# constantinpape/torch-em

Measured on AMD Instinct MI355X. Metric: voxels/sec fwd+bwd, UNet3d 1x128^3 bs=2, higher is better.
Workload: dtype f32-class (forward convs on normalised activations: fp32 operands split into 2 fp16 terms = 22 mantissa bits, lo plane scaled by 2^12 with its own fp32 accumulator, 3 fp16 MFMAs per product; other forward convs 3 bf16 terms / 6 MFMAs; data-gradient convs 2 bf16 terms / 3 MFMAs (16-bit products); WEI

## Files before the change

### torch_em_amd/csrc/capi.hip

```cpp
#include "tem_common.h"
#include "conv_internal.h"
#include "tem_act.h"
#include <stdarg.h>
#include <string.h>

static thread_local char g_err[512] = "";

void tem_set_error(const char* fmt, ...) {
    va_list ap;
    va_start(ap, fmt);
    vsnprintf(g_err, sizeof(g_err), fmt, ap);
    va_end(ap);
}

extern "C" const char* tem_last_error(void) { return g_err; }

struct TemOption {
    const char* name;
    long long def;
};
static const TemOption g_opt_table[TEM_OPT_COUNT] = {
    {"wgrad_zs", 3},
    {"wgrad_zs_persist", 1},
    {"wgrad_sums", 1},
    {"wgrad_sums_min_mb", 128},
    {"fwd_persistent", -1},
    {"conv_fwd_variant", -1},
    {"conv1x1_stream", 1},
    {"fwd_ksplit_chunks", 0},
    {"wgrad_cus", 256},
    {"upsample_generic", 0},
    {"team_min_units", 0},
    {"zr_splitk", 1},
    {"zr_wide", 1},
    {"zr_tile_blocks", 1},
    {"dice_vox", 1},
    {"upsample2_ch8", 1},
    {"pool_vec8", 2},
    {"fp32_zr", 1},
};
static long long g_opt_val[TEM_OPT_COUNT];
static bool g_opt_set[TEM_OPT_COUNT];

long long tem_option(int id) {
    if (id < 0 || id >= TEM_OPT_COUNT) return 0;
    return __atomic_load_n(&g_opt_set[id], __ATOMIC_RELAXED) ? __atomic_load_n(&g_opt_val[id], __ATOMIC_RELAXED)
                                                            : g_opt_table[id].def;
}
static int opt_find(const char* name) {
    if (!name) return -1;
    for (int i = 0; i < TEM_OPT_COUNT; ++i)
        if (!strcmp(name, g_opt_table[i].name)) return i;
    return -1;
}
extern "C" int tem_set_option(const char* name, int64_t value) {
    const int id = opt_find(name);
    TEM_REQUIRE(id >= 0, "tem_set_option: unknown option '%s'", name ? name : "(null)");
    __atomic_store_n(&g_opt_val[id], (long long)value, __ATOMIC_RELAXED);
    __atomic_store_n(&g_opt_set[id], true, __ATOMIC_RELAXED);
    return TEM_OK;
}
extern "C" int tem_get_option(const char* name, int64_t* value) {
    const int id = opt_find(name);
    TEM_REQUIRE(id >= 0 && value, "tem_get_option: unknown option '%s'", name ? name : "(null)");
    *value = (int64_t)tem_option(id);
    return TEM_OK;
}
extern "C" int tem_version(void) { return 100; }

extern "C" int tem_device_cus(void) {
    int dev = 0;
    if (hipGetDevice(&dev) != hipSuccess) return TEM_ELAUNCH;
    hipDeviceProp_t prop;
    if (hipGetDeviceProperties(&prop, dev) != hipSuccess) return TEM_ELAUNCH;
    return prop.multiProcessorCount;
}

#define TT_V 64
#define TT_C 32

__global__ __launch_bounds__(256) void k_nchw_to_nhwc(const float* __restrict__ src, float* __restrict__ dst,
                                                      int64_t dst_ld, int C, int64_t V, int64_t vtiles, int ctiles) {
    __shared__ float tile[TT_C][TT_V + 1];
    int64_t ntiles = vtiles * ctiles;
    int n = blockIdx.y;
    for (int64_t t = blockIdx.x; t < ntiles; t += gridDim.x) {
        int ct = (int)(t % ctiles);
        int64_t vt = t / ctiles;
        int64_t v0 = vt * TT_V;
        int c0 = ct * TT_C;
        for (int i = threadIdx.x; i < TT_C * TT_V; i += 256) {
            int c = i / TT_V, v = i % TT_V;
            float val = 0.f;
            if (c0 + c < C && v0 + v < V) val = src[((int64_t)n * C + c0 + c) * V + v0 + v];
            tile[c][v] = val;
        }
        __syncthreads();
        for (int i = threadIdx.x; i < TT_C * TT_V; i += 256) {
            int v = i / TT_C, c = i % TT_C;
            if (c0 + c < C && v0 + v < V) dst[((int64_t)n * V + v0 + v) * dst_ld + c0 + c] = tile[c][v];
        }
        __syncthreads();
    }
}

__global__ __launch_bounds__(256) void k_nhwc_to_nchw(const float* __restrict__ src, int64_t src_ld,
                                                      float* __restrict__ dst, int C, int64_t V, int64_t vtiles,
                                                      int ctiles) {
    __shared__ float tile[TT_C][TT_V + 1];
    int64_t ntiles = vtiles * ctiles;
    int n = blockIdx.y;
    for (int64_t t = blockIdx.x; t < ntiles; t += gridDim.x) {
        int ct = (int)(t % ctiles);
        int64_t vt = t / ctiles;
        int64_t v0 = vt * TT_V;
        int c0 = ct * TT_C;
        for (int i = threadIdx.x; i < TT_C * TT_V; i += 256) {
            int v = i / TT_C, c = i % TT_C;
            float val = 0.f;
            if (c0 + c < C && v0 + v < V) val = src[((int64_t)n * V + v0 + v) * src_ld + c0 + c];
            tile[c][v] = val;
        }
        __syncthreads();
        for (int i = threadIdx.x; i < TT_C * TT_V; i += 256) {
            int c = i / TT_V, v = i % TT_V;
            if (c0 + c < C && v0 + v < V) dst[((int64_t)n * C + c0 + c) * V + v0 + v] = tile[c][v];
        }
        __syncthreads();
    }
}

extern "C" int tem_nchw_to_nhwc(const float* src, float* dst, int64_t dst_ld, int N, int C, int64_t V,
                                tem_stream_t stream) {
    TEM_REQUIRE(src && dst && N > 0 && C > 0 && V > 0 && dst_ld >= C, "tem_nchw_to_nhwc: bad arguments");
    int64_t vtiles = tem_cdiv(V, TT_V);
    int ctiles = (int)tem_cdiv(C, TT_C);
    int64_t nt = vtiles * ctiles;
    dim3 grid((unsigned)(nt > 4096 ? 4096 : nt), N);
    hipLaunchKernelGGL(k_nchw_to_nhwc, grid, dim3(256), 0, (hipStream_t)stream, src, dst, dst_ld, C, V, vtiles, ctiles);
    TEM_CHECK_LAUNCH("tem_nchw_to_nhwc");
    return TEM_OK;
}

extern "C" int tem_nhwc_to_nchw(const float* src, int64_t src_ld, float* dst, int N, int C, int64_t V,
                                tem_stream_t stream) {
    TEM_REQUIRE(src && dst && N > 0 && C > 0 && V > 0 && src_ld >= C, "tem_nhwc_to_nchw: bad arguments");
    int64_t vtiles = tem_cdiv(V, TT_V);
    int ctiles = (int)tem_cdiv(C, TT_C);
    int64_t nt = vtiles * ctiles;
    dim3 grid((unsigned)(nt > 4096 ? 4096 : nt), N);
    hipLaunchKernelGGL(k_nhwc_to_nchw, grid, dim3(256), 0, (hipStream_t)stream, src, src_ld, dst, C, V, vtiles, ctiles);
    TEM_CHECK_LAUNCH("tem_nhwc_to_nchw");
    return TEM_OK;
}

#define STD_BLOCKS 256

__global__ __launch_bounds__(256) void k_std_partial(const float* __restrict__ x, int64_t L, double* __restrict__ part) {
    int n = blockIdx.y;
    const float* row = x + (int64_t)n * L;
    double s = 0.0, ss = 0.0;
    for (int64_t i = (int64_t)blockIdx.x * 256 + threadIdx.x; i < L; i += (int64_t)gridDim.x * 256) {
        double v = (double)row[i];
        s += v;
        ss += v * v;
    }
    s = tem_wave_sum_d(s);
    ss = tem_wave_sum_d(ss);
    __shared__ double sh[2][4];
    int w = threadIdx.x >> 6;
    if ((threadIdx.x & 63) == 0) { sh[0][w] = s; sh[1][w] = ss; }
    __syncthreads();
    if (threadIdx.x == 0) {
        part[((int64_t)n * gridDim.x + blockIdx.x) * 2 + 0] = sh[0][0] + sh[0][1] + sh[0][2] + sh[0][3];
        part[((int64_t)n * gridDim.x + blockIdx.x) * 2 + 1] = sh[1][0] + sh[1][1] + sh[1][2] + sh[1][3];
    }
}

__global__ __launch_bounds__(256) void k_std_apply(const float* __restrict__ x, float* __restrict__ y, int64_t L,
                                                   const double* __restrict__ part, int nblk, float eps) {
    int n = blockIdx.y;
    __shared__ float sh_mean, sh_inv;
    if (threadIdx.x == 0) {
        double s = 0.0, ss = 0.0;
        for (int b = 0; b < nblk; ++b) {
            s += part[((int64_t)n * nblk + b) * 2 + 0];
            ss += part[((int64_t)n * nblk + b) * 2 + 1];
        }
        double mean = s / (double)L;
        double var = ss / (double)L - mean * mean;
        if (var < 0.0) var = 0.0;
        sh_mean = (float)mean;
        sh_inv = (float)(1.0 / (sqrt(var) + (double)eps));
    }
    __syncthreads();
    float mean = sh_mean, inv = sh_inv;
    const float* row = x + (int64_t)n * L;
    float* out = y + (int64_t)n * L;
    for (int64_t i = (int64_t)blockIdx.x * 256 + threadIdx.x; i < L; i += (int64_t)gridDim.x * 256)
        out[i] = (row[i] - mean) * inv;
}

extern "C" int tem_standardize(const float* x, float* y, int N, int64_t L, float eps, void* ws, int64_t ws_bytes,
                               tem_stream_t stream) {
    TEM_REQUIRE(x && y && ws && N > 0 && L > 0, "tem_standardize: bad arguments");
    int nblk = (int)(tem_cdiv(L, 256) < STD_BLOCKS ? tem_cdiv(L, 256) : STD_BLOCKS);
    if ((int64_t)N * nblk * 2 * (int64_t)sizeof(double) > ws_bytes) {
        tem_set_error("tem_standardize: workspace too small (%lld bytes needed)",
                      (long long)((int64_t)N * nblk * 2 * sizeof(double)));
        return TEM_EWS;
    }
    hipLaunchKernelGGL(k_std_partial, dim3(nblk, N), dim3(256), 0, (hipStream_t)stream, x, L, (double*)ws);
    hipLaunchKernelGGL(k_std_apply, dim3(nblk, N), dim3(256), 0, (hipStream_t)stream, x, y, L, (const double*)ws, nblk, eps);
    TEM_CHECK_LAUNCH("tem_standardize");
    return TEM_OK;
}

__global__ __launch_bounds__(256) void k_act_bwd(const float* __restrict__ gy, const float* __restrict__ y,
                                                 float* __restrict__ gx, int64_t n, int act) {
    for (int64_t i = (int64_t)blockIdx.x * 256 + threadIdx.x; i < n; i += (int64_t)gridDim.x * 256) {
        float yv = y[i], g = gy[i];
        gx[i] = (act == TEM_ACT_SIGMOID) ? g * yv * (1.f - yv) : ((yv > 0.f) ? g : 0.f);
    }
}

extern "C" int tem_act_bwd(const float* gy, const float* y, float* gx, int64_t n, int act, tem_stream_t stream) {
    TEM_REQUIRE(gy && y && gx && n > 0, "tem_act_bwd: bad arguments");
    TEM_REQUIRE(act == TEM_ACT_RELU || act == TEM_ACT_SIGMOID, "tem_act_bwd: Invalid activation: %d", act);
    hipLaunchKernelGGL(k_act_bwd, dim3(tem_grid_1d(n, 256)), dim3(256), 0, (hipStream_t)stream, gy, y, gx, n, act);
    TEM_CHECK_LAUNCH("tem_act_bwd");
    return TEM_OK;
}
```

### torch_em_amd/csrc/pool_upsample.hip

```cpp
#include "tem_common.h"
#include "tem_act.h"

template <int VEC>
struct VecT;
template <>
struct VecT<4> {
    typedef float4 type;
};
template <>
struct VecT<1> {
    typedef float type;
};

template <int VEC, typename T>
__device__ __forceinline__ void ld_vec(const T* p, float (&v)[VEC]) {
    if constexpr (VEC == 8) {
        act_ld8(p, v);
    } else if constexpr (VEC == 4) {
        const float4 t = act_ld4(p);
        v[0] = t.x; v[1] = t.y; v[2] = t.z; v[3] = t.w;
    } else {
        v[0] = act_ld1(p);
    }
}
// ... 555 lines not shown
                }
            ++cnt;
        }
    }
    return cnt;
}

__device__ __forceinline__ void utu_axis(int i, int f, int in, float (&a)[3], float& s) {
    a[0] = a[1] = a[2] = 0.f;
    s = 0.f;
    const int olo = max(0, f * i - f), ohi = min(in * f - 1, f * i + 2 * f - 1);
    for (int o = olo; o <= ohi; ++o) {
        const float w = lin_w(o, f, in, i);
        if (w == 0.f) continue;
        s += w;
#pragma unroll
        for (int d = -1; d <= 1; ++d)
            if (i + d >= 0 && i + d < in) a[d + 1] = fmaf(w, lin_w(o, f, in, i + d), a[d + 1]);
    }
}

template <int VEC, typename T>
__global__ __launch_bounds__(256) void k_upsample_bwd(const T* __restrict__ gy, int64_t gy_ld,
                                                      T* __restrict__ gx, int64_t gx_ld, int D, int H, int W, int C,
                                                      int fz, int fy, int fx, const T* __restrict__ u, int64_t u_ld,
                                                      const float* __restrict__ ncoef, int64_t ncoef_ld) {
    const int Do = D * fz, Ho = H * fy, Wo = W * fx;
    const int cq = C / VEC;
    int row = blockIdx.x;
    const int yi = row % H;
    row /= H;
    const int zi = row % D;
    const int n = row / D;
    const int zlo = max(0, fz * zi - fz), zhi = min(Do - 1, fz * zi + 2 * fz - 1);
    const int ylo = max(0, fy * yi - fy), yhi = min(Ho - 1, fy * yi + 2 * fy - 1);
    const bool fast = fz <= 2 && fy <= 2 && fx <= 2;
    int zidx[4], yidx[4];
    float zw[4], yw[4];
    int nzt = 0;
    if (fast) {
        nzt = upb_taps(zlo, zhi, fz, D, zi, zidx, zw);
        upb_taps(ylo, yhi, fy, H, yi, yidx, yw);
    }
    float az[3] = {0.f, 0.f, 0.f}, ay[3] = {0.f, 0.f, 0.f}, sz = 0.f, sy = 0.f;
    if (ncoef) {
        utu_axis(zi, fz, D, az, sz);
        utu_axis(yi, fy, H, ay, sy);
    }
    for (int i = threadIdx.x; i < W * cq; i += 256) {
        const int xi = i / cq, c0 = (i % cq) * VEC;
        const int xlo = max(0, fx * xi - fx), xhi = min(Wo - 1, fx * xi + 2 * fx - 1);
        float acc[VEC];
#pragma unroll
        for (int j = 0; j < VEC; ++j) acc[j] = 0.f;
        if (fast) {
            int xidx[4];
            float xw[4];
            upb_taps(xlo, xhi, fx, W, xi, xidx, xw);
            for (int kz = 0; kz < nzt; ++kz) {
                const int64_t rz = ((int64_t)n * Do + zidx[kz]) * Ho;
                float t[4][4][VEC];
#pragma unroll
                for (int ky = 0; ky < 4; ++ky)
#pragma unroll
                    for (int kx = 0; kx < 4; ++kx) ld_vec<VEC>(gy + ((rz + yidx[ky]) * Wo + xidx[kx]) * gy_ld + c0, t[ky][kx]);
#pragma unroll
                for (int ky = 0; ky < 4; ++ky)
#pragma unroll
                    for (int kx = 0; kx < 4; ++kx) {
                        const float w = zw[kz] * yw[ky] * xw[kx];
#pragma unroll
                        for (int j = 0; j < VEC; ++j) acc[j] = fmaf(w, t[ky][kx][j], acc[j]);
                    }
            }
        } else
        for (int zo = zlo; zo <= zhi; ++zo) {
            float wz = lin_w(zo, fz, D, zi);
            if (wz == 0.f) continue;
            for (int yo = ylo; yo <= yhi; ++yo) {
                float wy = lin_w(yo, fy, H, yi);
                if (wy == 0.f) continue;
                const int64_t r = (((int64_t)n * Do + zo) * Ho + yo) * Wo;
                for (int xo = xlo; xo <= xhi; ++xo) {
                    float wx = lin_w(xo, fx, W, xi);
                    if (wx == 0.f) continue;
                    float t[VEC];
                    ld_vec<VEC>(gy + (r + xo) * gy_ld + c0, t);
                    const float w = wz * wy * wx;
#pragma unroll
                    for (int j = 0; j < VEC; ++j) acc[j] = fmaf(w, t[j], acc[j]);
                }
            }
        }
        int64_t v = (((int64_t)n * D + zi) * H + yi) * W + xi;
        if (ncoef) {
            float ax[3], sx;
            utu_axis(xi, fx, W, ax, sx);
            const float S = sz * sy * sx;
            float q[VEC];
#pragma unroll
            for (int j = 0; j < VEC; ++j) q[j] = 0.f;
#pragma unroll
            for (int dz = -1; dz <= 1; ++dz) {
                const int zc = min(max(zi + dz, 0), D - 1);
                float t[3][3][VEC];
#pragma unroll
                for (int dy = -1; dy <= 1; ++dy) {
                    const int yc = min(max(yi + dy, 0), H - 1);
#pragma unroll
                    for (int dx = -1; dx <= 1; ++dx) {
                        const int xc = min(max(xi + dx, 0), W - 1);
                        ld_vec<VEC>(u + ((((int64_t)n * D + zc) * H + yc) * W + xc) * u_ld + c0, t[dy + 1][dx + 1]);
                    }
                }
#pragma unroll
                for (int dy = -1; dy <= 1; ++dy)
#pragma unroll
                    for (int dx = -1; dx <= 1; ++dx) {
                        const float wq = az[dz + 1] * ay[dy + 1] * ax[dx + 1];
#pragma unroll
                        for (int j = 0; j < VEC; ++j) q[j] = fmaf(wq, t[dy + 1][dx + 1][j], q[j]);
                    }
            }
#pragma unroll
            for (int j = 0; j < VEC; ++j) {
                const float4 kc = *reinterpret_cast<const float4*>(ncoef + (int64_t)n * ncoef_ld + (c0 + j) * 4);
                acc[j] = kc.x * acc[j] - kc.y * S - kc.z * (q[j] - kc.w * S);
            }
        }
        st_vec<VEC>(gx + v * gx_ld + c0, acc);
    }
}

template <int CH>
struct FV {
    float v[CH];
};
template <int CH, typename T>
__device__ __forceinline__ FV<CH> ldv(const T* p) {
    FV<CH> r;
    if constexpr (CH == 8) {
        act_ld8(p, r.v);
    } else {
        const float4 t = act_ld4(p);
        r.v[0] = t.x; r.v[1] = t.y; r.v[2] = t.z; r.v[3] = t.w;
    }
    return r;
}
template <int CH, typename T>
__device__ __forceinline__ void stv(T* p, const FV<CH>& a) {
    if constexpr (CH == 8) act_st8(p, a.v);
    else act_st4(p, make_float4(a.v[0], a.v[1], a.v[2], a.v[3]));
}
template <int CH>
__device__ __forceinline__ FV<CH> fv_zero() {
    FV<CH> r;
#pragma unroll
    for (int j = 0; j < CH; ++j) r.v[j] = 0.f;
    return r;
}
template <int CH>
__device__ __forceinline__ FV<CH> lerp2(float l0, const FV<CH>& a, float l1, const FV<CH>& b) {
    FV<CH> r;
#pragma unroll
    for (int j = 0; j < CH; ++j) r.v[j] = l0 * a.v[j] + l1 * b.v[j];
    return r;
}

template <int FZ, typename T, int CH = 4>
__global__ __launch_bounds__(256) void k_upsample2_fwd(const T* __restrict__ x, int64_t x_ld, T* __restrict__ y,
                                                       int64_t y_ld, int D, int H, int W, int C,
                                                       float* __restrict__ part) {
    extern __shared__ float lsu[];
    const int Ho = 2 * H, Wo = 2 * W;
    const int cq = C / CH;
    int row = blockIdx.x;
    const int yi = row % H;
    row /= H;
    const int zi = row % D;
    const int n = row / D;
    const int ym = max(yi - 1, 0), yp = min(yi + 1, H - 1);
    const int zm = max(zi - 1, 0), zp = min(zi + 1, D - 1);
    const float ya0 = yi == 0 ? 1.f : 0.25f, ya1 = yi == 0 ? 0.f : 0.75f;
    const float za0 = zi == 0 ? 1.f : 0.25f, za1 = zi == 0 ? 0.f : 0.75f;
    const int zrow[3] = {zm, zi, zp}, yrow[3] = {ym, yi, yp};
    float s1[CH], s2[CH];
#pragma unroll
    for (int j = 0; j < CH; ++j) s1[j] = s2[j] = 0.f;
    for (int i = threadIdx.x; i < W * cq; i += 256) {
        const int xi = i / cq, c0 = (i % cq) * CH;
        const int xm = max(xi - 1, 0), xp = min(xi + 1, W - 1);
        const float xa0 = xi == 0 ? 1.f : 0.25f, xa1 = xi == 0 ? 0.f : 0.75f;
        FV<CH> Y[FZ == 2 ? 3 : 1][2][2];
#pragma unroll
        for (int kz = 0; kz < (FZ == 2 ? 3 : 1); ++kz) {
            const int zc = FZ == 2 ? zrow[kz] : zi;
            FV<CH> X[3][2];
#pragma unroll
            for (int ky = 0; ky < 3; ++ky) {
                const T* r = x + ((((int64_t)n * D + zc) * H + yrow[ky]) * W) * x_ld + c0;
                const FV<CH> a = ldv<CH>(r + (int64_t)xm * x_ld), b = ldv<CH>(r + (int64_t)xi * x_ld), c = ldv<CH>(r + (int64_t)xp * x_ld);
                X[ky][0] = lerp2(xa0, a, xa1, b);
                X[ky][1] = lerp2(0.75f, b, 0.25f, c);
            }
#pragma unroll
            for (int sx = 0; sx < 2; ++sx) {
                Y[kz][0][sx] = lerp2(ya0, X[0][sx], ya1, X[1][sx]);
                Y[kz][1][sx] = lerp2(0.75f, X[1][sx], 0.25f, X[2][sx]);
            }
            __builtin_amdgcn_sched_barrier(0);
        }
#pragma unroll
        for (int sz = 0; sz < FZ; ++sz)
#pragma unroll
            for (int sy = 0; sy < 2; ++sy)
#pragma unroll
                for (int sx = 0; sx < 2; ++sx) {
                    FV<CH> o;
                    if constexpr (FZ == 2)
                        o = sz == 0 ? lerp2(za0, Y[0][sy][sx], za1, Y[1][sy][sx]) : lerp2(0.75f, Y[1][sy][sx], 0.25f, Y[2][sy][sx]);
                    else
                        o = Y[0][sy][sx];
                    const int64_t vo = (((int64_t)n * (D * FZ) + zi * FZ + sz) * Ho + 2 * yi + sy) * Wo + 2 * xi + sx;
                    if constexpr (sizeof(T) == 2) {
#pragma unroll
                        for (int j = 0; j < CH; j += 2) {
                            const unsigned pk = act_pk<T>(o.v[j], o.v[j + 1]);
                            o.v[j] = act_lo<T>(pk);
                            o.v[j + 1] = act_hi<T>(pk);
                        }
                    }
                    stv<CH>(y + vo * y_ld + c0, o);
#pragma unroll
                    for (int j = 0; j < CH; ++j) {
                        s1[j] += o.v[j];
                        s2[j] = fmaf(o.v[j], o.v[j], s2[j]);
                    }
                }
    }
    if (part) {
        const int wv = threadIdx.x >> 6, lane = threadIdx.x & 63;
#pragma unroll
        for (int j = 0; j < CH; ++j) {
            for (int o = cq; o < 64; o <<= 1) {
                s1[j] += __shfl_xor(s1[j], o, 64);
                s2[j] += __shfl_xor(s2[j], o, 64);
            }
            if (lane < cq) {
                lsu[(wv * C + lane * CH + j) * 2 + 0] = s1[j];
                lsu[(wv * C + lane * CH + j) * 2 + 1] = s2[j];
            }
        }
        __syncthreads();
        for (int t = threadIdx.x; t < 2 * C; t += 256) {
            float a = 0.f;
            for (int w4 = 0; w4 < 4; ++w4) a += lsu[w4 * 2 * C + t];
            part[((int64_t)n * D * H + (int64_t)zi * H + yi) * 2 * C + t] = a;
        }
    }
}

struct UpbAxis {
    int idx[6];
    float w[2][4];
};
__device__ __forceinline__ UpbAxis upb_axis2(int i0, int in) {
    UpbAxis a;
    const int out = 2 * in;
#pragma unroll
    for (int k = 0; k < 6; ++k) a.idx[k] = min(max(2 * i0 - 1 + k, 0), out - 1);
#pragma unroll
    for (int c = 0; c < 2; ++c)
#pragma unroll
        for (int k = 0; k < 4; ++k) {
            const int o = 2 * i0 - 1 + 2 * c + k;
            a.w[c][k] = (o >= 0 && o < out && i0 + c < in) ? lin_w(o, 2, in, i0 + c) : 0.f;
        }
    return a;
}
__device__ __forceinline__ float upb_w(int o, int in, int i) {
    return (o >= 0 && o < 2 * in && i < in) ? lin_w(o, 2, in, i) : 0.f;
}
__device__ __forceinline__ float pick3(const float (&a)[3], int d) {
    return d == 0 ? a[0] : d == 1 ? a[1] : d == 2 ? a[2] : 0.f;
}
struct UtuAxis {
    int idx[4];
    float a[2][3];
    float s[2];
};
__device__ __forceinline__ UtuAxis utu_axis2(int i0, int f, int in) {
    UtuAxis r;
#pragma unroll
    for (int k = 0; k < 4; ++k) r.idx[k] = min(max(i0 - 1 + k, 0), in - 1);
#pragma unroll
    for (int c = 0; c < 2; ++c) {
        r.a[c][0] = r.a[c][1] = r.a[c][2] = 0.f;
        r.s[c] = 0.f;
        if (i0 + c < in) utu_axis(i0 + c, f, in, r.a[c], r.s[c]);
    }
    return r;
}

template <int FZ, typename T, int CH = 4>
__global__ __launch_bounds__(256) void k_upsample2_bwd(const T* __restrict__ gy, int64_t gy_ld,
                                                       T* __restrict__ gx, int64_t gx_ld, int D, int H, int W, int C,
                                                       const T* __restrict__ u, int64_t u_ld,
                                                       const float* __restrict__ ncoef, int64_t ncoef_ld) {
    constexpr int CZ = FZ == 2 ? 2 : 1;
    constexpr int NZF = FZ == 2 ? 6 : 1;
    const int Do = D * FZ, Ho = 2 * H, Wo = 2 * W;
    const int cq = C / CH;
    const int Hp = (H + 1) >> 1, Wp = (W + 1) >> 1, Dp = (D + CZ - 1) / CZ;
    int row = blockIdx.x;
    const int y0 = (row % Hp) * 2;
    row /= Hp;
    const int z0 = (row % Dp) * CZ;
    const int n = row / Dp;
    for (int i = threadIdx.x; i < Wp * cq; i += 256) {
        const int x0 = (i / cq) * 2, c0 = (i % cq) * CH;
        const UpbAxis ax = upb_axis2(x0, W);
        FV<CH> acc[CZ][2][2];
#pragma unroll
        for (int a = 0; a < CZ; ++a)
#pragma unroll
            for (int b = 0; b < 2; ++b)
#pragma unroll
                for (int c = 0; c < 2; ++c) acc[a][b][c] = fv_zero<CH>();
#pragma unroll 1
        for (int kz = 0; kz < NZF; ++kz) {
            const int oz = FZ == 2 ? 2 * z0 - 1 + kz : z0;
            const int zf = min(max(oz, 0), Do - 1);
            float wz[CZ];
#pragma unroll
            for (int a = 0; a < CZ; ++a) wz[a] = FZ == 2 ? upb_w(oz, D, z0 + a) : 1.f;
            FV<CH> pp[2][2];
#pragma unroll
            for (int b = 0; b < 2; ++b)
#pragma unroll
                for (int c = 0; c < 2; ++c) pp[b][c] = fv_zero<CH>();
#pragma unroll 2
            for (int ky = 0; ky < 6; ++ky) {
                const int oy = 2 * y0 - 1 + ky;
                const float wy[2] = {upb_w(oy, H, y0), upb_w(oy, H, y0 + 1)};
                const T* r = gy + ((((int64_t)n * Do + zf) * Ho + min(max(oy, 0), Ho - 1)) * Wo) * gy_ld + c0;
                FV<CH> t[6];
#pragma unroll
                for (int kx = 0; kx < 6; ++kx) t[kx] = ldv<CH>(r + (int64_t)ax.idx[kx] * gy_ld);
#pragma unroll
                for (int c = 0; c < 2; ++c)
#pragma unroll
                    for (int j = 0; j < CH; ++j) {
                        const float xr = ax.w[c][0] * t[2 * c].v[j] + ax.w[c][1] * t[2 * c + 1].v[j] +
                                         ax.w[c][2] * t[2 * c + 2].v[j] + ax.w[c][3] * t[2 * c + 3].v[j];
                        pp[0][c].v[j] = fmaf(wy[0], xr, pp[0][c].v[j]);
                        pp[1][c].v[j] = fmaf(wy[1], xr, pp[1][c].v[j]);
                    }
            }
#pragma unroll
            for (int a = 0; a < CZ; ++a)
#pragma unroll
                for (int b = 0; b < 2; ++b)
#pragma unroll
                    for (int c = 0; c < 2; ++c)
#pragma unroll
                        for (int j = 0; j < CH; ++j) acc[a][b][c].v[j] = fmaf(wz[a], pp[b][c].v[j], acc[a][b][c].v[j]);
        }
        if (ncoef) {
            const UtuAxis bx = utu_axis2(x0, 2, W), by = utu_axis2(y0, 2, H), bz = utu_axis2(z0, FZ, D);
            FV<CH> q[CZ][2][2];
#pragma unroll
            for (int a = 0; a < CZ; ++a)
#pragma unroll
                for (int b = 0; b < 2; ++b)
#pragma unroll
                    for (int c = 0; c < 2; ++c) q[a][b][c] = fv_zero<CH>();
            constexpr int NZU = FZ == 2 ? 4 : 1;
#pragma unroll 1
            for (int kz = 0; kz < NZU; ++kz) {
                const int zc = FZ == 2 ? min(max(z0 - 1 + kz, 0), D - 1) : z0;
                float wz[CZ];
#pragma unroll
                for (int a = 0; a < CZ; ++a) wz[a] = FZ == 2 ? pick3(bz.a[a], kz - a) : 1.f;
                FV<CH> qp[2][2];
#pragma unroll
                for (int b = 0; b < 2; ++b)
#pragma unroll
                    for (int c = 0; c < 2; ++c) qp[b][c] = fv_zero<CH>();
#pragma unroll 2
                for (int ky = 0; ky < 4; ++ky) {
                    const float wy[2] = {pick3(by.a[0], ky), pick3(by.a[1], ky - 1)};
                    const T* r = u + ((((int64_t)n * D + zc) * H + min(max(y0 - 1 + ky, 0), H - 1)) * W) * u_ld + c0;
                    FV<CH> t[4];
#pragma unroll
                    for (int kx = 0; kx < 4; ++kx) t[kx] = ldv<CH>(r + (int64_t)bx.idx[kx] * u_ld);
#pragma unroll
                    for (int c = 0; c < 2; ++c)
#pragma unroll
                        for (int j = 0; j < CH; ++j) {
                            const float xr = bx.a[c][0] * t[c].v[j] + bx.a[c][1] * t[c + 1].v[j] + bx.a[c][2] * t[c + 2].v[j];
                            qp[0][c].v[j] = fmaf(wy[0], xr, qp[0][c].v[j]);
                            qp[1][c].v[j] = fmaf(wy[1], xr, qp[1][c].v[j]);
                        }
                }
#pragma unroll
                for (int a = 0; a < CZ; ++a)
#pragma unroll
                    for (int b = 0; b < 2; ++b)
#pragma unroll
                        for (int c = 0; c < 2; ++c)
#pragma unroll
                            for (int j = 0; j < CH; ++j) q[a][b][c].v[j] = fmaf(wz[a], qp[b][c].v[j], q[a][b][c].v[j]);
            }
            float4 kc[CH];
#pragma unroll
            for (int j = 0; j < CH; ++j) kc[j] = *reinterpret_cast<const float4*>(ncoef + (int64_t)n * ncoef_ld + (c0 + j) * 4);
#pragma unroll
            for (int a = 0; a < CZ; ++a)
#pragma unroll
                for (int b = 0; b < 2; ++b)
#pragma unroll
                    for (int c = 0; c < 2; ++c) {
                        const float S = (FZ == 2 ? bz.s[a] : 1.f) * by.s[b] * bx.s[c];
#pragma unroll
                        for (int j = 0; j < CH; ++j)
                            acc[a][b][c].v[j] = kc[j].x * acc[a][b][c].v[j] - kc[j].y * S - kc[j].z * (q[a][b][c].v[j] - kc[j].w * S);
                    }
        }
#pragma unroll
        for (int a = 0; a < CZ; ++a)
#pragma unroll
            for (int b = 0; b < 2; ++b)
#pragma unroll
                for (int c = 0; c < 2; ++c) {
                    if (z0 + a >= D || y0 + b >= H || x0 + c >= W) continue;
                    const int64_t v = (((int64_t)n * D + z0 + a) * H + y0 + b) * W + x0 + c;
                    stv<CH>(gx + v * gx_ld + c0, acc[a][b][c]);
                }
    }
}

template <int VEC, typename T>
__global__ __launch_bounds__(256) void k_upsample_stats(const T* __restrict__ u, int64_t u_ld, int D, int H, int W,
                                                        int C, int fz, int fy, int fx, float* __restrict__ part) {
    extern __shared__ float lsu[];
    const int cq = C / VEC;
    int row = blockIdx.x;
    const int yi = row % H;
    row /= H;
    const int zi = row % D;
    const int n = row / D;
    float az[3], ay[3], sz, sy;
    utu_axis(zi, fz, D, az, sz);
    utu_axis(yi, fy, H, ay, sy);
    float s1[VEC], s2[VEC];
#pragma unroll
    for (int j = 0; j < VEC; ++j) s1[j] = s2[j] = 0.f;
    for (int i = threadIdx.x; i < W * cq; i += 256) {
        const int xi = i / cq, c0 = (i % cq) * VEC;
        float ax[3], sx;
        utu_axis(xi, fx, W, ax, sx);
        const float S = sz * sy * sx;
        float q[VEC], uc[VEC];
#pragma unroll
        for (int j = 0; j < VEC; ++j) q[j] = 0.f;
        ld_vec<VEC>(u + ((((int64_t)n * D + zi) * H + yi) * W + xi) * u_ld + c0, uc);
#pragma unroll
        for (int dz = -1; dz <= 1; ++dz) {
            const int zc = min(max(zi + dz, 0), D - 1);
            float t[3][3][VEC];
#pragma unroll
            for (int dy = -1; dy <= 1; ++dy) {
                const int yc = min(max(yi + dy, 0), H - 1);
#pragma unroll
                for (int dx = -1; dx <= 1; ++dx) {
                    const int xc = min(max(xi + dx, 0), W - 1);
                    ld_vec<VEC>(u + ((((int64_t)n * D + zc) * H + yc) * W + xc) * u_ld + c0, t[dy + 1][dx + 1]);
                }
            }
#pragma unroll
            for (int dy = -1; dy <= 1; ++dy)
#pragma unroll
                for (int dx = -1; dx <= 1; ++dx) {
                    const float wq = az[dz + 1] * ay[dy + 1] * ax[dx + 1];
#pragma unroll
                    for (int j = 0; j < VEC; ++j) q[j] = fmaf(wq, t[dy + 1][dx + 1][j], q[j]);
                }
        }
#pragma unroll
        for (int j = 0; j < VEC; ++j) {
            s1[j] = fmaf(S, uc[j], s1[j]);
            s2[j] = fmaf(uc[j], q[j], s2[j]);
        }
    }
    const int wv = threadIdx.x >> 6, lane = threadIdx.x & 63;
#pragma unroll
    for (int j = 0; j < VEC; ++j) {
        for (int o = cq; o < 64; o <<= 1) {
            s1[j] += __shfl_xor(s1[j], o, 64);
            s2[j] += __shfl_xor(s2[j], o, 64);
        }
        if (lane < cq) {
            lsu[(wv * C + lane * VEC + j) * 2 + 0] = s1[j];
            lsu[(wv * C + lane * VEC + j) * 2 + 1] = s2[j];
        }
    }
    __syncthreads();
    for (int t = threadIdx.x; t < 2 * C; t += 256) {
        float a = 0.f;
        for (int w4 = 0; w4 < 4; ++w4) a += lsu[w4 * 2 * C + t];
        part[((int64_t)n * D * H + (int64_t)zi * H + yi) * 2 * C + t] = a;
    }
}

static int upsample_stats_impl(const void* u, int64_t u_ld, int N, int D, int H, int W, int C, int fz, int fy, int fx,
                               float* part, int st, tem_stream_t stream) {
    TEM_REQUIRE(u && part && N > 0 && C > 0 && u_ld >= C && D > 0 && H > 0 && W > 0 && fz > 0 && fy > 0 && fx > 0,
                "tem_upsample_stats: bad arguments");
    TEM_REQUIRE(st >= 0 && st <= 2, "tem_upsample_stats: unknown storage type %d", st);
    const int cq = C / 4;
    TEM_REQUIRE(C % 4 == 0 && cq <= 64 && (cq & (cq - 1)) == 0 && u_ld % 4 == 0 && ((uintptr_t)u % tem_st_align4(st) == 0),
                "tem_upsample_stats: needs C = 4 * 2^k <= 256 channels, rows aligned to 4 elements (got C=%d)", C);
    int64_t rows = (int64_t)N * D * H;
    TEM_REQUIRE(rows < (1ll << 31), "tem_upsample_stats: too many rows");
    TEM_ST_SWITCH(st, T, hipLaunchKernelGGL((k_upsample_stats<4, T>), dim3((unsigned)rows), dim3(256), (size_t)4 * C * 2 * sizeof(float),
                                            (hipStream_t)stream, (const T*)u, u_ld, D, H, W, C, fz, fy, fx, part));
    TEM_CHECK_LAUNCH("tem_upsample_stats");
    return TEM_OK;
}
extern "C" int tem_upsample_stats(const float* u, int64_t u_ld, int N, int D, int H, int W, int C, int fz, int fy, int fx,
                                  float* part, tem_stream_t stream) {
    return upsample_stats_impl(u, u_ld, N, D, H, W, C, fz, fy, fx, part, 0, stream);
}
extern "C" int tem_upsample_stats_st(const void* u, int64_t u_ld, int N, int D, int H, int W, int C, int fz, int fy, int fx,
                                     float* part, int st, tem_stream_t stream) {
    return upsample_stats_impl(u, u_ld, N, D, H, W, C, fz, fy, fx, part, st, stream);
}

static inline bool upsample2_ok(int C, int fz, int fy, int fx) {
    return fy == 2 && fx == 2 && (fz == 1 || fz == 2) && C % 4 == 0 && !tem_option(TEM_OPT_UPSAMPLE_GENERIC);
}

extern "C" int tem_upsample_fwd_stats_ok(int C, int fz, int fy, int fx) {
    const int cq = C / 4;
    return upsample2_ok(C, fz, fy, fx) && cq <= 64 && (cq & (cq - 1)) == 0;
}

static int upsample_fwd_impl(const void* x, int64_t x_ld, void* y, int64_t y_ld, int N, int D, int H, int W, int C, int fz,
                             int fy, int fx, float* part, int st, tem_stream_t stream) {
    TEM_REQUIRE(x && y && N > 0 && C > 0 && x_ld >= C && y_ld >= C && D > 0 && H > 0 && W > 0,
                "tem_upsample_fwd: bad arguments");
    TEM_REQUIRE(st >= 0 && st <= 2, "tem_upsample_fwd: unknown storage type %d", st);
    TEM_REQUIRE(fz > 0 && fy > 0 && fx > 0, "tem_upsample_fwd: bad factors");
    const bool v4 = vec4_ok(C, {x, y}, {x_ld, y_ld}, st);
    TEM_REQUIRE(!part || (tem_upsample_fwd_stats_ok(C, fz, fy, fx) && v4),
                "tem_upsample_fwd_stats: needs factors (1|2, 2, 2), C = 4 * 2^k <= 256 and rows aligned to 4 elements");
    int64_t rows = (int64_t)N * D * fz * H * fy;
    TEM_REQUIRE(rows < (1ll << 31), "tem_upsample_fwd: too many rows");
    const size_t ldsb = part ? (size_t)4 * C * 2 * sizeof(float) : 0;
    if (fz == 1 && upsample2_ok(C, fz, fy, fx) && vec8_ok(C, {x, y}, {x_ld, y_ld}, st) && ((C / 8) & (C / 8 - 1)) == 0 && C / 8 <= 64) {
        const int64_t crow = (int64_t)N * D * H;
        TEM_ST16_SWITCH(st, T, {
            hipLaunchKernelGGL((k_upsample2_fwd<1, T, 8>), dim3((unsigned)crow), dim3(256), ldsb, (hipStream_t)stream, (const T*)x,
                               x_ld, (T*)y, y_ld, D, H, W, C, part);
        });
        TEM_CHECK_LAUNCH("tem_upsample_fwd");
        return TEM_OK;
    }
    TEM_ST_SWITCH(st, T, {
        const T* xs = (const T*)x;
        T* ys = (T*)y;
        if (upsample2_ok(C, fz, fy, fx) && v4) {
            const int64_t crow = (int64_t)N * D * H;
            if (fz == 2)
                hipLaunchKernelGGL((k_upsample2_fwd<2, T>), dim3((unsigned)crow), dim3(256), ldsb, (hipStream_t)stream, xs, x_ld, ys,
                                   y_ld, D, H, W, C, part);
            else
                hipLaunchKernelGGL((k_upsample2_fwd<1, T>), dim3((unsigned)crow), dim3(256), ldsb, (hipStream_t)stream, xs, x_ld, ys,
                                   y_ld, D, H, W, C, part);
        } else if (v4)
            hipLaunchKernelGGL((k_upsample_fwd<4, T>), dim3((unsigned)rows), dim3(256), 0, (hipStream_t)stream, xs, x_ld, ys,
                               y_ld, D, H, W, C, fz, fy, fx);
        else
            hipLaunchKernelGGL((k_upsample_fwd<1, T>), dim3((unsigned)rows), dim3(256), 0, (hipStream_t)stream, xs, x_ld, ys,
                               y_ld, D, H, W, C, fz, fy, fx);
    });
    TEM_CHECK_LAUNCH("tem_upsample_fwd");
    return TEM_OK;
}

extern "C" int tem_upsample_fwd_stats(const float* x, int64_t x_ld, float* y, int64_t y_ld, int N, int D, int H, int W,
                                      int C, int fz, int fy, int fx, float* part, tem_stream_t stream) {
    TEM_REQUIRE(part, "tem_upsample_fwd_stats: bad arguments");
    return upsample_fwd_impl(x, x_ld, y, y_ld, N, D, H, W, C, fz, fy, fx, part, 0, stream);
}

extern "C" int tem_upsample_fwd(const float* x, int64_t x_ld, float* y, int64_t y_ld, int N, int D, int H, int W, int C,
                                int fz, int fy, int fx, tem_stream_t stream) {
    return upsample_fwd_impl(x, x_ld, y, y_ld, N, D, H, W, C, fz, fy, fx, nullptr, 0, stream);
}

extern "C" int tem_upsample_fwd_st(const void* x, int64_t x_ld, void* y, int64_t y_ld, int N, int D, int H, int W, int C,
                                   int fz, int fy, int fx, float* part, int st, tem_stream_t stream) {
    return upsample_fwd_impl(x, x_ld, y, y_ld, N, D, H, W, C, fz, fy, fx, part, st, stream);
}

static int upsample_bwd_impl(const void* gy, int64_t gy_ld, void* gx, int64_t gx_ld, int N, int D, int H, int W,
                             int C, int fz, int fy, int fx, const void* u, int64_t u_ld, const float* ncoef,
                             int64_t ncoef_ld, int st, tem_stream_t stream) {
    TEM_REQUIRE(gy && gx && N > 0 && C > 0 && gy_ld >= C && gx_ld >= C && D > 0 && H > 0 && W > 0,
                "tem_upsample_bwd: bad arguments");
    TEM_REQUIRE(st >= 0 && st <= 2, "tem_upsample_bwd: unknown storage type %d", st);
    TEM_REQUIRE(fz > 0 && fy > 0 && fx > 0, "tem_upsample_bwd: bad factors");
    int64_t rows = (int64_t)N * D * H;
    TEM_REQUIRE(rows < (1ll << 31), "tem_upsample_bwd: too many rows");
    const int64_t pairs = (int64_t)N * ((D + fz - 1) / fz) * ((H + 1) / 2) * ((W + 1) / 2) * (C / 4);
    if (upsample2_ok(C, fz, fy, fx) && pairs >= 2 * 65536 && vec8_ok(C, {gy, gx, u}, {gy_ld, gx_ld, u ? u_ld : 0}, st) && tem_option(TEM_OPT_UPSAMPLE2_CH8)) {
        TEM_ST16_SWITCH(st, T, {
            if (fz == 2) {
                const int64_t prow = (int64_t)N * ((D + 1) / 2) * ((H + 1) / 2);
                hipLaunchKernelGGL((k_upsample2_bwd<2, T, 8>), dim3((unsigned)prow), dim3(256), 0, (hipStream_t)stream, (const T*)gy,
                                   gy_ld, (T*)gx, gx_ld, D, H, W, C, (const T*)u, u_ld, ncoef, ncoef_ld);
            } else {
                const int64_t prow = (int64_t)N * D * ((H + 1) / 2);
                hipLaunchKernelGGL((k_upsample2_bwd<1, T, 8>), dim3((unsigned)prow), dim3(256), 0, (hipStream_t)stream, (const T*)gy,
                                   gy_ld, (T*)gx, gx_ld, D, H, W, C, (const T*)u, u_ld, ncoef, ncoef_ld);
            }
        });
        TEM_CHECK_LAUNCH("tem_upsample_bwd");
        return TEM_OK;
    }
    TEM_ST_SWITCH(st, T, {
        const T* gys = (const T*)gy;
        const T* us = (const T*)u;
        T* gxs = (T*)gx;
        if (upsample2_ok(C, fz, fy, fx) && pairs >= 65536 && vec4_ok(C, {gy, gx, u}, {gy_ld, gx_ld, u_ld}, st)) {
            if (fz == 2) {
                const int64_t prow = (int64_t)N * ((D + 1) / 2) * ((H + 1) / 2);
                hipLaunchKernelGGL((k_upsample2_bwd<2, T>), dim3((unsigned)prow), dim3(256), 0, (hipStream_t)stream, gys, gy_ld, gxs,
                                   gx_ld, D, H, W, C, us, u_ld, ncoef, ncoef_ld);
            } else {
                const int64_t prow = (int64_t)N * D * ((H + 1) / 2);
                hipLaunchKernelGGL((k_upsample2_bwd<1, T>), dim3((unsigned)prow), dim3(256), 0, (hipStream_t)stream, gys, gy_ld, gxs,
                                   gx_ld, D, H, W, C, us, u_ld, ncoef, ncoef_ld);
            }
        } else if (vec4_ok(C, {gy, gx, u}, {gy_ld, gx_ld, u ? u_ld : 0}, st))
            hipLaunchKernelGGL((k_upsample_bwd<4, T>), dim3((unsigned)rows), dim3(256), 0, (hipStream_t)stream, gys, gy_ld, gxs,
                               gx_ld, D, H, W, C, fz, fy, fx, us, u_ld, ncoef, ncoef_ld);
        else
            hipLaunchKernelGGL((k_upsample_bwd<1, T>), dim3((unsigned)rows), dim3(256), 0, (hipStream_t)stream, gys, gy_ld, gxs,
                               gx_ld, D, H, W, C, fz, fy, fx, us, u_ld, ncoef, ncoef_ld);
    });
    TEM_CHECK_LAUNCH("tem_upsample_bwd");
    return TEM_OK;
}

extern "C" int tem_upsample_bwd(const float* gy, int64_t gy_ld, float* gx, int64_t gx_ld, int N, int D, int H, int W,
                                int C, int fz, int fy, int fx, tem_stream_t stream) {
    return upsample_bwd_impl(gy, gy_ld, gx, gx_ld, N, D, H, W, C, fz, fy, fx, nullptr, 0, nullptr, 0, 0, stream);
}

extern "C" int tem_upsample_bwd_norm(const float* gy, int64_t gy_ld, float* gx, int64_t gx_ld, int N, int D, int H,
                                     int W, int C, int fz, int fy, int fx, const float* u, int64_t u_ld,
                                     const float* ncoef, int64_t ncoef_ld, tem_stream_t stream) {
    TEM_REQUIRE(u && ncoef, "tem_upsample_bwd_norm: bad arguments");
    return tem_upsample_bwd_st(gy, gy_ld, gx, gx_ld, N, D, H, W, C, fz, fy, fx, u, u_ld, ncoef, ncoef_ld, TEM_ST_F32, stream);
}

extern "C" int tem_upsample_bwd_st(const void* gy, int64_t gy_ld, void* gx, int64_t gx_ld, int N, int D, int H, int W, int C,
                                   int fz, int fy, int fx, const void* u, int64_t u_ld, const float* ncoef, int64_t ncoef_ld,
                                   int st, tem_stream_t stream) {
    TEM_REQUIRE((u == nullptr) == (ncoef == nullptr), "tem_upsample_bwd_norm: u and ncoef come together");
    if (ncoef) {
        TEM_REQUIRE(u_ld >= C && ncoef_ld >= 4 * C && ((uintptr_t)ncoef % 16 == 0) && ncoef_ld % 4 == 0,
                    "tem_upsample_bwd_norm: bad arguments");
        TEM_REQUIRE(st >= 0 && st <= 2 && (C % 4 || (u_ld % 4 == 0 && (uintptr_t)u % tem_st_align4(st) == 0)),
                    "tem_upsample_bwd_norm: u must be aligned to 4 elements");
    }
    return upsample_bwd_impl(gy, gy_ld, gx, gx_ld, N, D, H, W, C, fz, fy, fx, u, u_ld, ncoef, ncoef_ld, st, stream);
}
```

### torch_em_amd/csrc/tem_common.h

```cpp
#pragma once
#include <hip/hip_runtime.h>
#include <stdint.h>
#include <stdio.h>
#include "../../include/tem_hip.h"

void tem_set_error(const char* fmt, ...);

enum {
    TEM_OPT_WGRAD_ZS = 0,
    TEM_OPT_WGRAD_ZS_PERSIST,
    TEM_OPT_WGRAD_SUMS,
    TEM_OPT_WGRAD_SUMS_MIN_MB,
    TEM_OPT_FWD_PERSISTENT,
    TEM_OPT_CONV_FWD_VARIANT,
    TEM_OPT_CONV1X1_STREAM,
    TEM_OPT_FWD_KSPLIT_CHUNKS,
    TEM_OPT_WGRAD_CUS,
    TEM_OPT_UPSAMPLE_GENERIC,
    TEM_OPT_TEAM_MIN_UNITS,
    TEM_OPT_ZR_SPLITK,
    TEM_OPT_ZR_WIDE,
    TEM_OPT_ZR_TILE_BLOCKS,
    TEM_OPT_DICE_VOX,
    TEM_OPT_UPSAMPLE2_CH8,
    TEM_OPT_POOL_VEC8,
    TEM_OPT_FP32_ZR,
    TEM_OPT_COUNT
};
long long tem_option(int id);

#define TEM_REQUIRE(cond, ...)                 \
    do {                                       \
        if (!(cond)) {                         \
            tem_set_error(__VA_ARGS__);        \
            return TEM_EINVAL;                 \
        }                                      \
    } while (0)

#define TEM_TRY(call)                          \
    do {                                       \
        const int rc__ = (call);               \
        if (rc__ != TEM_OK) return rc__;       \
    } while (0)

#define TEM_CHECK_LAUNCH(name)                                                   \
    do {                                                                         \
        hipError_t e__ = hipGetLastError();                                      \
        if (e__ != hipSuccess) {                                                 \
            tem_set_error("%s: launch failed: %s", name, hipGetErrorString(e__)); \
            return TEM_ELAUNCH;                                                  \
        }                                                                        \
    } while (0)

static inline int64_t tem_cdiv(int64_t a, int64_t b) { return (a + b - 1) / b; }
static inline int64_t tem_align_up(int64_t a, int64_t b) { return tem_cdiv(a, b) * b; }

static inline int tem_grid_1d(int64_t work_items, int block, int max_blocks = 256 * 8) {
    int64_t g = tem_cdiv(work_items, block);
    if (g > max_blocks) g = max_blocks;
    if (g < 1) g = 1;
    return (int)g;
}

#define TEM_WAVE 64

__device__ __forceinline__ float tem_amax4(float m, float a, float b, float c, float d) {
    return __builtin_fmaxf(__builtin_fmaxf(m, __builtin_fmaxf(__builtin_fabsf(a), __builtin_fabsf(b))),
                           __builtin_fmaxf(__builtin_fabsf(c), __builtin_fabsf(d)));
}
__device__ __forceinline__ void tem_amax_commit(unsigned* amax, float m) {
    unsigned u = __builtin_bit_cast(unsigned, m);
#pragma unroll
    for (int o = 32; o > 0; o >>= 1) u = max(u, (unsigned)__shfl_xor((int)u, o, 64));
    if ((threadIdx.x & 63) == 0 && u > __atomic_load_n(amax, __ATOMIC_RELAXED)) atomicMax(amax, u);
}

__device__ __forceinline__ float tem_wave_sum(float v) {
#pragma unroll
    for (int o = 32; o > 0; o >>= 1) v += __shfl_xor(v, o, 64);
    return v;
}
__device__ __forceinline__ double tem_wave_sum_d(double v) {
#pragma unroll
    for (int o = 32; o > 0; o >>= 1) v += __shfl_xor(v, o, 64);
    return v;
}

__device__ __forceinline__ int tem_xcd_remap(int bid, int nwg) {
    const int nx = 8;
    int q = nwg / nx, r = nwg % nx;
    int xcd = bid % nx, idx = bid / nx;
    int base = (xcd < r) ? xcd * (q + 1) : r * (q + 1) + (xcd - r) * q;
    return base + idx;
}
```

Before: 278.6 million.

## Add z-marching trilinear upsample backward kernel reusing output-plane partial sums

Adds a new upsample-by-2 backward kernel in which each block marches along z over a segment of depth. Each fine output plane's y/x-reduced partial sum is computed once and applied to both neighbouring coarse planes through rolling lo/hi accumulators. The old kernel read 6 fine planes per coarse pair, so overlapping planes were read twice. The segment length is picked on the host so there are enough blocks to fill the GPU, and the kernel uses XCD remapping. A few expressions are also rewritten as explicit fmaf chains, and a min_pairs option is added. The cost is fewer, longer-running blocks and a serial z loop with more branching.

```diff
diff --git a/torch_em_amd/csrc/capi.hip b/torch_em_amd/csrc/capi.hip
--- a/torch_em_amd/csrc/capi.hip
+++ b/torch_em_amd/csrc/capi.hip
@@ -38,6 +38,8 @@
     {"upsample2_ch8", 1},
     {"pool_vec8", 2},
     {"fp32_zr", 1},
+    {"upsample2_march", 1},
+    {"upsample2_min_pairs", 65536},
 };
 static long long g_opt_val[TEM_OPT_COUNT];
 static bool g_opt_set[TEM_OPT_COUNT];
diff --git a/torch_em_amd/csrc/pool_upsample.hip b/torch_em_amd/csrc/pool_upsample.hip
--- a/torch_em_amd/csrc/pool_upsample.hip
+++ b/torch_em_amd/csrc/pool_upsample.hip
@@ -881,6 +881,65 @@
     return r;
 }
 
+__device__ __forceinline__ float upb_xrow4(const float (&w)[4], float t0, float t1, float t2, float t3) {
+    return fmaf(w[3], t3, fmaf(w[2], t2, fmaf(w[0], t0, __fmul_rn(w[1], t1))));
+}
+__device__ __forceinline__ float utu_xrow3(const float (&a)[3], float t0, float t1, float t2) {
+    return fmaf(a[2], t2, fmaf(a[0], t0, __fmul_rn(a[1], t1)));
+}
+__device__ __forceinline__ float upb_norm_tail(const float4& kc, float acc, float q, float S) {
+    return fmaf(-kc.z, fmaf(-kc.w, S, q), fmaf(kc.x, acc, -__fmul_rn(kc.y, S)));
+}
+template <int CH, typename T>
+__device__ __forceinline__ void upb_plane(const T* __restrict__ gy, int64_t gy_ld, int64_t zrow, int Ho, int Wo, int y0, int H,
+                                          int c0, const UpbAxis& ax, FV<CH> (&pp)[2][2]) {
+#pragma unroll
+    for (int b = 0; b < 2; ++b)
+#pragma unroll
+        for (int c = 0; c < 2; ++c) pp[b][c] = fv_zero<CH>();
+#pragma unroll 2
+    for (int ky = 0; ky < 6; ++ky) {
+        const int oy = 2 * y0 - 1 + ky;
+        const float wy[2] = {upb_w(oy, H, y0), upb_w(oy, H, y0 + 1)};
+        const T* r = gy + ((zrow + min(max(oy, 0), Ho - 1)) * Wo) * gy_ld + c0;
+        FV<CH> t[6];
+#pragma unroll
+        for (int kx = 0; kx < 6; ++kx) t[kx] = ldv<CH>(r + (int64_t)ax.idx[kx] * gy_ld);
+#pragma unroll
+        for (int c = 0; c < 2; ++c)
+#pragma unroll
+            for (int j = 0; j < CH; ++j) {
+                const float xr = upb_xrow4(ax.w[c], t[2 * c].v[j], t[2 * c + 1].v[j], t[2 * c + 2].v[j], t[2 * c + 3].v[j]);
+                pp[0][c].v[j] = fmaf(wy[0], xr, pp[0][c].v[j]);
+                pp[1][c].v[j] = fmaf(wy[1], xr, pp[1][c].v[j]);
+            }
+    }
+}
+template <int CH, typename T>
+__device__ __forceinline__ void utu_plane(const T* __restrict__ u, int64_t u_ld, int64_t zrow, int H, int W, int y0, int c0,
+                                          const UtuAxis& bx, const UtuAxis& by, FV<CH> (&qp)[2][2]) {
+#pragma unroll
+    for (int b = 0; b < 2; ++b)
+#pragma unroll
+        for (int c = 0; c < 2; ++c) qp[b][c] = fv_zero<CH>();
+#pragma unroll 2
+    for (int ky = 0; ky < 4; ++ky) {
+        const float wy[2] = {pick3(by.a[0], ky), pick3(by.a[1], ky - 1)};
+        const T* r = u + ((zrow + min(max(y0 - 1 + ky, 0), H - 1)) * W) * u_ld + c0;
+        FV<CH> t[4];
+#pragma unroll
+        for (int kx = 0; kx < 4; ++kx) t[kx] = ldv<CH>(r + (int64_t)bx.idx[kx] * u_ld);
+#pragma unroll
+        for (int c = 0; c < 2; ++c)
+#pragma unroll
+            for (int j = 0; j < CH; ++j) {
+                const float xr = utu_xrow3(bx.a[c], t[c].v[j], t[c + 1].v[j], t[c + 2].v[j]);
+                qp[0][c].v[j] = fmaf(wy[0], xr, qp[0][c].v[j]);
+                qp[1][c].v[j] = fmaf(wy[1], xr, qp[1][c].v[j]);
+            }
+    }
+}
+
 template <int FZ, typename T, int CH = 4>
 __global__ __launch_bounds__(256) void k_upsample2_bwd(const T* __restrict__ gy, int64_t gy_ld,
                                                        T* __restrict__ gx, int64_t gx_ld, int D, int H, int W, int C,
@@ -914,28 +973,7 @@
 #pragma unroll
             for (int a = 0; a < CZ; ++a) wz[a] = FZ == 2 ? upb_w(oz, D, z0 + a) : 1.f;
             FV<CH> pp[2][2];
-#pragma unroll
-            for (int b = 0; b < 2; ++b)
-#pragma unroll
-                for (int c = 0; c < 2; ++c) pp[b][c] = fv_zero<CH>();
-#pragma unroll 2
-            for (int ky = 0; ky < 6; ++ky) {
-                const int oy = 2 * y0 - 1 + ky;
-                const float wy[2] = {upb_w(oy, H, y0), upb_w(oy, H, y0 + 1)};
-                const T* r = gy + ((((int64_t)n * Do + zf) * Ho + min(max(oy, 0), Ho - 1)) * Wo) * gy_ld + c0;
-                FV<CH> t[6];
-#pragma unroll
-                for (int kx = 0; kx < 6; ++kx) t[kx] = ldv<CH>(r + (int64_t)ax.idx[kx] * gy_ld);
-#pragma unroll
-                for (int c = 0; c < 2; ++c)
-#pragma unroll
-                    for (int j = 0; j < CH; ++j) {
-                        const float xr = ax.w[c][0] * t[2 * c].v[j] + ax.w[c][1] * t[2 * c + 1].v[j] +
-                                         ax.w[c][2] * t[2 * c + 2].v[j] + ax.w[c][3] * t[2 * c + 3].v[j];
-                        pp[0][c].v[j] = fmaf(wy[0], xr, pp[0][c].v[j]);
-                        pp[1][c].v[j] = fmaf(wy[1], xr, pp[1][c].v[j]);
-                    }
-            }
+            upb_plane<CH>(gy, gy_ld, ((int64_t)n * Do + zf) * Ho, Ho, Wo, y0, H, c0, ax, pp);
 #pragma unroll
             for (int a = 0; a < CZ; ++a)
 #pragma unroll
@@ -962,26 +1000,7 @@
 #pragma unroll
                 for (int a = 0; a < CZ; ++a) wz[a] = FZ == 2 ? pick3(bz.a[a], kz - a) : 1.f;
                 FV<CH> qp[2][2];
-#pragma unroll
-                for (int b = 0; b < 2; ++b)
-#pragma unroll
-                    for (int c = 0; c < 2; ++c) qp[b][c] = fv_zero<CH>();
-#pragma unroll 2
-                for (int ky = 0; ky < 4; ++ky) {
-                    const float wy[2] = {pick3(by.a[0], ky), pick3(by.a[1], ky - 1)};
-                    const T* r = u + ((((int64_t)n * D + zc) * H + min(max(y0 - 1 + ky, 0), H - 1)) * W) * u_ld + c0;
-                    FV<CH> t[4];
-#pragma unroll
-                    for (int kx = 0; kx < 4; ++kx) t[kx] = ldv<CH>(r + (int64_t)bx.idx[kx] * u_ld);
-#pragma unroll
-                    for (int c = 0; c < 2; ++c)
-#pragma unroll
-                        for (int j = 0; j < CH; ++j) {
-                            const float xr = bx.a[c][0] * t[c].v[j] + bx.a[c][1] * t[c + 1].v[j] + bx.a[c][2] * t[c + 2].v[j];
-                            qp[0][c].v[j] = fmaf(wy[0], xr, qp[0][c].v[j]);
-                            qp[1][c].v[j] = fmaf(wy[1], xr, qp[1][c].v[j]);
-                        }
-                }
+                utu_plane<CH>(u, u_ld, ((int64_t)n * D + zc) * H, H, W, y0, c0, bx, by, qp);
 #pragma unroll
                 for (int a = 0; a < CZ; ++a)
 #pragma unroll
@@ -1003,7 +1022,7 @@
                         const float S = (FZ == 2 ? bz.s[a] : 1.f) * by.s[b] * bx.s[c];
 #pragma unroll
                         for (int j = 0; j < CH; ++j)
-                            acc[a][b][c].v[j] = kc[j].x * acc[a][b][c].v[j] - kc[j].y * S - kc[j].z * (q[a][b][c].v[j] - kc[j].w * S);
+                            acc[a][b][c].v[j] = upb_norm_tail(kc[j], acc[a][b][c].v[j], q[a][b][c].v[j], S);
                     }
         }
 #pragma unroll
@@ -1016,6 +1035,107 @@
                     const int64_t v = (((int64_t)n * D + z0 + a) * H + y0 + b) * W + x0 + c;
                     stv<CH>(gx + v * gx_ld + c0, acc[a][b][c]);
                 }
+    }
+}
+
+template <typename T, int CH = 4>
+__global__ __launch_bounds__(256) void k_upsample2_march(const T* __restrict__ gy, int64_t gy_ld,
+                                                         T* __restrict__ gx, int64_t gx_ld, int D, int H, int W, int C,
+                                                         const T* __restrict__ u, int64_t u_ld,
+                                                         const float* __restrict__ ncoef, int64_t ncoef_ld, int S) {
+    const int Do = 2 * D, Ho = 2 * H, Wo = 2 * W;
+    const int cq = C / CH;
+    const int Hp = (H + 1) >> 1, Wp = (W + 1) >> 1, nseg = (D + 2 * S - 1) / (2 * S);
+    int row = tem_xcd_remap(blockIdx.x, gridDim.x);
+    const int y0 = (row % Hp) * 2;
+    row /= Hp;
+    const int zs = (row % nseg) * 2 * S, ze = min(zs + 2 * S, D) - 1;
+    const int n = row / nseg;
+    const int oz_first = max(2 * zs - 1, 0), oz_last = min(2 * ze + 2, Do - 1);
+    for (int i = threadIdx.x; i < Wp * cq; i += 256) {
+        const int x0 = (i / cq) * 2, c0 = (i % cq) * CH;
+        const UpbAxis ax = upb_axis2(x0, W);
+        FV<CH> lo[2][2], hi[2][2];
+#pragma unroll
+        for (int b = 0; b < 2; ++b)
+#pragma unroll
+            for (int c = 0; c < 2; ++c) lo[b][c] = hi[b][c] = fv_zero<CH>();
+#pragma unroll 1
+        for (int oz = oz_first; oz <= oz_last; ++oz) {
+            FV<CH> pp[2][2];
+            upb_plane<CH>(gy, gy_ld, ((int64_t)n * Do + oz) * Ho, Ho, Wo, y0, H, c0, ax, pp);
+            const int chi = (oz + 1) >> 1, clo = chi - 1;
+            if (clo >= zs) {
+                const float wz = upb_w(oz, D, clo);
+#pragma unroll
+                for (int b = 0; b < 2; ++b)
+#pragma unroll
+                    for (int c = 0; c < 2; ++c)
+#pragma unroll
+                        for (int j = 0; j < CH; ++j) lo[b][c].v[j] = fmaf(wz, pp[b][c].v[j], lo[b][c].v[j]);
+            }
+            if (chi <= ze) {
+                const float wz = upb_w(oz, D, chi);
+#pragma unroll
+                for (int b = 0; b < 2; ++b)
+#pragma unroll
+                    for (int c = 0; c < 2; ++c)
+#pragma unroll
+                        for (int j = 0; j < CH; ++j) hi[b][c].v[j] = fmaf(wz, pp[b][c].v[j], hi[b][c].v[j]);
+            }
+            if ((oz & 1) && oz != Do - 1) continue;
+            if (clo >= zs) {
+                if (ncoef) {
+                    const UtuAxis bx = utu_axis2(x0, 2, W), by = utu_axis2(y0, 2, H);
+                    float az[3], sz;
+                    utu_axis(clo, 2, D, az, sz);
+                    FV<CH> q[2][2];
+#pragma unroll
+                    for (int b = 0; b < 2; ++b)
+#pragma unroll
+                        for (int c = 0; c < 2; ++c) q[b][c] = fv_zero<CH>();
+#pragma unroll 1
+                    for (int d = 0; d < 3; ++d) {
+                        const int zc = min(max(clo - 1 + d, 0), D - 1);
+                        const float wz = pick3(az, d);
+                        FV<CH> qp[2][2];
+                        utu_plane<CH>(u, u_ld, ((int64_t)n * D + zc) * H, H, W, y0, c0, bx, by, qp);
+#pragma unroll
+                        for (int b = 0; b < 2; ++b)
+#pragma unroll
+                            for (int c = 0; c < 2; ++c)
+#pragma unroll
+                                for (int j = 0; j < CH; ++j) q[b][c].v[j] = fmaf(wz, qp[b][c].v[j], q[b][c].v[j]);
+                    }
+                    float4 kc[CH];
+#pragma unroll
+                    for (int j = 0; j < CH; ++j) kc[j] = *reinterpret_cast<const float4*>(ncoef + (int64_t)n * ncoef_ld + (c0 + j) * 4);
+#pragma unroll
+                    for (int b = 0; b < 2; ++b)
+#pragma unroll
+                        for (int c = 0; c < 2; ++c) {
+                            const float Sw = sz * by.s[b] * bx.s[c];
+#pragma unroll
+                            for (int j = 0; j < CH; ++j) lo[b][c].v[j] = upb_norm_tail(kc[j], lo[b][c].v[j], q[b][c].v[j], Sw);
+                        }
+                }
+#pragma unroll
+                for (int b = 0; b < 2; ++b)
+#pragma unroll
+                    for (int c = 0; c < 2; ++c) {
+                        if (y0 + b >= H || x0 + c >= W) continue;
+                        const int64_t v = (((int64_t)n * D + clo) * H + y0 + b) * W + x0 + c;
+                        stv<CH>(gx + v * gx_ld + c0, lo[b][c]);
+                    }
+            }
+#pragma unroll
+            for (int b = 0; b < 2; ++b)
+#pragma unroll
+                for (int c = 0; c < 2; ++c) {
+                    lo[b][c] = hi[b][c];
+                    hi[b][c] = fv_zero<CH>();
+                }
+        }
     }
 }
 
@@ -1194,9 +1314,19 @@
     int64_t rows = (int64_t)N * D * H;
     TEM_REQUIRE(rows < (1ll << 31), "tem_upsample_bwd: too many rows");
     const int64_t pairs = (int64_t)N * ((D + fz - 1) / fz) * ((H + 1) / 2) * ((W + 1) / 2) * (C / 4);
-    if (upsample2_ok(C, fz, fy, fx) && pairs >= 2 * 65536 && vec8_ok(C, {gy, gx, u}, {gy_ld, gx_ld, u ? u_ld : 0}, st) && tem_option(TEM_OPT_UPSAMPLE2_CH8)) {
+    const int64_t min_pairs = tem_option(TEM_OPT_UPSAMPLE2_MIN_PAIRS);
+    const long long march = fz == 2 ? tem_option(TEM_OPT_UPSAMPLE2_MARCH) : 0;
+    const int Dp2 = (D + 1) / 2, Hp2 = (H + 1) / 2;
+    int seg = march >= 2 ? (int)(march < Dp2 ? march : Dp2) : 4;
+    if (march == 1)
+        while (seg > 1 && (int64_t)N * ((Dp2 + seg - 1) / seg) * Hp2 < 2 * 256) seg >>= 1;
+    const int64_t mrow = (int64_t)N * ((Dp2 + seg - 1) / seg) * Hp2;
+    if (upsample2_ok(C, fz, fy, fx) && pairs >= 2 * min_pairs && vec8_ok(C, {gy, gx, u}, {gy_ld, gx_ld, u ? u_ld : 0}, st) && tem_option(TEM_OPT_UPSAMPLE2_CH8)) {
         TEM_ST16_SWITCH(st, T, {
-            if (fz == 2) {
+            if (march) {
+                hipLaunchKernelGGL((k_upsample2_march<T, 8>), dim3((unsigned)mrow), dim3(256), 0, (hipStream_t)stream, (const T*)gy,
+                                   gy_ld, (T*)gx, gx_ld, D, H, W, C, (const T*)u, u_ld, ncoef, ncoef_ld, seg);
+            } else if (fz == 2) {
                 const int64_t prow = (int64_t)N * ((D + 1) / 2) * ((H + 1) / 2);
                 hipLaunchKernelGGL((k_upsample2_bwd<2, T, 8>), dim3((unsigned)prow), dim3(256), 0, (hipStream_t)stream, (const T*)gy,
                                    gy_ld, (T*)gx, gx_ld, D, H, W, C, (const T*)u, u_ld, ncoef, ncoef_ld);
@@ -1213,8 +1343,11 @@
         const T* gys = (const T*)gy;
         const T* us = (const T*)u;
         T* gxs = (T*)gx;
-        if (upsample2_ok(C, fz, fy, fx) && pairs >= 65536 && vec4_ok(C, {gy, gx, u}, {gy_ld, gx_ld, u_ld}, st)) {
-            if (fz == 2) {
+        if (upsample2_ok(C, fz, fy, fx) && pairs >= min_pairs && vec4_ok(C, {gy, gx, u}, {gy_ld, gx_ld, u_ld}, st)) {
+            if (march) {
+                hipLaunchKernelGGL((k_upsample2_march<T>), dim3((unsigned)mrow), dim3(256), 0, (hipStream_t)stream, gys, gy_ld, gxs,
+                                   gx_ld, D, H, W, C, us, u_ld, ncoef, ncoef_ld, seg);
+            } else if (fz == 2) {
                 const int64_t prow = (int64_t)N * ((D + 1) / 2) * ((H + 1) / 2);
                 hipLaunchKernelGGL((k_upsample2_bwd<2, T>), dim3((unsigned)prow), dim3(256), 0, (hipStream_t)stream, gys, gy_ld, gxs,
                                    gx_ld, D, H, W, C, us, u_ld, ncoef, ncoef_ld);
diff --git a/torch_em_amd/csrc/tem_common.h b/torch_em_amd/csrc/tem_common.h
--- a/torch_em_amd/csrc/tem_common.h
+++ b/torch_em_amd/csrc/tem_common.h
@@ -25,6 +25,8 @@
     TEM_OPT_UPSAMPLE2_CH8,
     TEM_OPT_POOL_VEC8,
     TEM_OPT_FP32_ZR,
+    TEM_OPT_UPSAMPLE2_MARCH,
+    TEM_OPT_UPSAMPLE2_MIN_PAIRS,
     TEM_OPT_COUNT
 };
 long long tem_option(int id);
```

Result: no change. 278.4 million (-0.1%).
